# xwhan/ProQA

Hardware: AMD Instinct MI355X
Metric: queries/sec top-80 MIPS over 18M x 128 index (higher is better)
Workload: dtype int8 nomination + f16 re-scoring; 1 GPU; top-80 MIPS, 2032 q x 18000000 x 128 fp16 rows in HBM (BASELINE configs[2]; x1 row shards: co...; rows=18000000, queries=2032, topk=80, parallelism=corpus-row-shard x1, exchange=none, rounds=4, fallback_rounds=0, leap_rank=33, world_size=1

## Files before the change

### proqa_amd/csrc/mips_index.cpp

```cpp
#include <algorithm>
#include <cmath>
#include <cstdio>
#include <cstdlib>
#include <cstring>
#include <condition_variable>
#include <mutex>
#include <new>
#include <thread>
#include <vector>

#include <fcntl.h>
#include <unistd.h>
#include <cerrno>

#include "common.h"
#include "mips_kernels.h"

namespace proqa {

struct Slab {
  long long r0, r1;
};

}
// ... 1291 lines not shown
      log_line("index %p: a leaping round found fewer than k rows above its threshold or overflowed (%d overflow-safe rounds, overflow "
               "bits %u): ordinary rounds for the next %d searches", (void*)idx, idx->stats.fallback_rounds, idx->overflow_bits,
               idx->leap_skip);
    } else {
      log_line("index %p: a leaping round found fewer than k rows above its threshold for %zu quer%s: leaps go on (%d strikes of 8)",
               (void*)idx, idx->rescue.ids.size(), idx->rescue.ids.size() == 1 ? "y" : "ies", idx->leap_strikes);
    }
  } else {
    if (idx->leap_strikes > 0) --idx->leap_strikes;
    if (idx->leap_pause) {
      log_line("index %p: leaping rounds resumed", (void*)idx);
      idx->leap_pause = 0;
    }
  }
  idx->stats.leap_state = leap_state_of(idx);
}

int finish_pending(proqa_index* idx, int* rewritten);
int search_device_impl(proqa_index* idx, const void* xq_dev, int64_t nq, int dtype, int k, int64_t idx_offset, float* D_dev,
                       int64_t* I_dev, hipStream_t st, bool defer, uint32_t* status_dev);

int rescue_short_queries(proqa_index* idx) {
  proqa_index::Rescue rq;
  std::swap(rq, idx->rescue);
  const int s = (int)rq.ids.size(), k = rq.k;
  if (s == 0) return PROQA_OK;
  const size_t off_xq = round_up<size_t>((size_t)s * sizeof(int), 256), off_d = off_xq + (size_t)s * kDim * 2,
               off_i = round_up<size_t>(off_d + (size_t)s * k * sizeof(float), 256), bytes = off_i + (size_t)s * k * sizeof(long long);
  if (bytes > idx->rescue_bytes) {
    if (idx->rescue_buf) (void)hipFree(idx->rescue_buf);
  if (idx->emit_log) (void)hipFree(idx->emit_log);
  if (idx->emit_cnt) (void)hipFree(idx->emit_cnt);
    idx->rescue_buf = nullptr;
    idx->rescue_bytes = 0;
    PROQA_HIP(hipMalloc(&idx->rescue_buf, bytes));
    idx->rescue_bytes = bytes;
  }
  char* base = (char*)idx->rescue_buf;
  int* ids_dev = (int*)base;
  float* D_tmp = (float*)(base + off_d);
  long long* I_tmp = (long long*)(base + off_i);
  PROQA_HIP(hipMemcpyAsync(ids_dev, rq.ids.data(), (size_t)s * sizeof(int), hipMemcpyHostToDevice, rq.st));
  PROQA_HIP(launch_gather_query_rows(idx->xq_pad, ids_dev, s, base + off_xq, rq.st));
  const proqa_search_stats outer = idx->stats;
  const int mode = idx->leap_mode;
  idx->leap_mode = 0;
  const bool unprofitable = idx->q8_unprofitable, small_ok = idx->small_merge_ok;
  const int suspended = idx->q8_suspended_searches, probe_after = idx->q8_probe_after, on_copy = idx->q8_searches_on_copy;
  const int rc = search_device_impl(idx, base + off_xq, s, PROQA_F16, k, rq.idx_offset, D_tmp, (int64_t*)I_tmp, rq.st, false, nullptr);
  idx->leap_mode = mode;
  idx->q8_unprofitable = unprofitable;
  idx->small_merge_ok = small_ok;
  idx->q8_suspended_searches = suspended;
  idx->q8_probe_after = probe_after;
  idx->q8_searches_on_copy = on_copy;
  if (rc) return rc;
  PROQA_HIP(launch_scatter_result_rows(D_tmp, I_tmp, ids_dev, s, k, rq.D, rq.I, rq.out_stride, rq.st));
  PROQA_HIP(hipStreamSynchronize(rq.st));
  const proqa_search_stats inner = idx->stats;
  idx->stats = outer;
  idx->stats.fallback_rounds += inner.rounds + inner.fallback_rounds;
  idx->stats.candidates += inner.candidates;
  idx->stats.nominated += inner.nominated;
  idx->stats.total_ms += inner.total_ms;
  idx->stats.nomination_state = nomination_state_of(idx);
  idx->stats.leap_state = leap_state_of(idx);
  log_line("index %p: %d quer%s a leaping round left short searched again on ordinary rounds (%d rounds, %.3f ms)", (void*)idx, s,
           s == 1 ? "y" : "ies", inner.rounds, inner.total_ms);
  return PROQA_OK;
}

int search_device_impl_body(proqa_index* idx, const void* xq_dev, int64_t nq, int dtype, int k, int64_t idx_offset, float* D_dev,
                            int64_t* I_dev, hipStream_t st, bool defer, uint32_t* status_dev);

int search_device(proqa_index* idx, const void* xq_dev, int64_t nq, int dtype, int k, int64_t idx_offset,
                  float* D_dev, int64_t* I_dev, hipStream_t st, bool defer = false, uint32_t* status_dev = nullptr) {
  const int rc = search_device_impl(idx, xq_dev, nq, dtype, k, idx_offset, D_dev, I_dev, st, defer, status_dev);
#ifdef PROQA_FILTER_STAMPS
  {
    unsigned long long h[8];
    read_filter_stamps(h);
    if (h[4])
      fprintf(stderr, "filter stamps (one wave per workgroup, %llu workgroups over all launches of the search): per unit MFMA section %.1f "
              "ticks, test section %.1f ticks; units per wave %.0f, wave lifetime per unit %.1f ticks; int8 scan: barrier + DMA issue %.1f "
              "ticks per unit, %.3f excursions per unit of %.1f ticks each\n", h[4], (double)h[0] / h[2],
              (double)h[1] / h[2], (double)h[2] / h[4], (double)h[3] / h[2], (double)h[5] / h[2], (double)h[7] / h[2],
              h[7] ? (double)h[6] / h[7] : 0.0);
  }
#endif
  if (rc == PROQA_OK && status_dev && !idx->pending.active) PROQA_HIP(hipMemsetAsync(status_dev, 0, sizeof(uint32_t), st));
  return rc;
}

int search_device_impl(proqa_index* idx, const void* xq_dev, int64_t nq, int dtype, int k, int64_t idx_offset,
                       float* D_dev, int64_t* I_dev, hipStream_t st, bool defer, uint32_t* status_dev) {
  idx->rescue.ids.clear();
  if (int rc = search_device_impl_body(idx, xq_dev, nq, dtype, k, idx_offset, D_dev, I_dev, st, defer, status_dev)) return rc;
  return idx->rescue.ids.empty() ? PROQA_OK : rescue_short_queries(idx);
}

int search_device_impl_body(proqa_index* idx, const void* xq_dev, int64_t nq, int dtype, int k, int64_t idx_offset,
                            float* D_dev, int64_t* I_dev, hipStream_t st, bool defer, uint32_t* status_dev) {
  if (idx->pending.active)
    if (int rc = finish_pending(idx, nullptr)) return rc;
  if (nq < 0 || k <= 0) return fail(PROQA_EINVAL, "search: nq=%lld k=%d", (long long)nq, k);
  if (dtype != PROQA_F16 && dtype != PROQA_F32) return fail(PROQA_EINVAL, "search: bad dtype %d", dtype);
  if (idx->n >= (1ll << 32)) return fail(PROQA_EINVAL, "search: shard has >= 2^32 rows");
  idx->stats = {};
  idx->stats.nomination_state = nomination_state_of(idx);
  idx->stats.leap_state = leap_state_of(idx);
  idx->q8_active = false;
  idx->pending_nq = nq;
  idx->used_small_merge = false;
  idx->overflow_bits = 0;
  idx->leap_active = false;
  if (nq == 0) return PROQA_OK;
  PROQA_ON_DEVICE(idx->device);

  const int qw = nq > 256 ? 2 : 1;
  const unsigned tile_q = filter_tile_queries(qw);
  const unsigned n_qtiles = (unsigned)ceil_div<int64_t>(nq, tile_q);
  const int64_t nq_pad = (int64_t)n_qtiles * tile_q;
  const int page_size = k <= kPageK ? kPageK : kBigPageK;
  OnePassPlan one_pass = plan_one_pass(idx, nq_pad, k, qw == 1);
  if (one_pass.use && nq_pad > one_pass.max_queries) {
    const size_t esize = dtype == PROQA_F16 ? 2 : 4;
    proqa_search_stats sum = {};
    const int64_t n_groups = ceil_div<int64_t>(nq, one_pass.max_queries);
    const int64_t per_group = round_up<int64_t>(ceil_div<int64_t>(nq, n_groups), 512);
    for (int64_t q0 = 0; q0 < nq; q0 += per_group) {
      const int64_t m = std::min<int64_t>(per_group, nq - q0);
      if (int rc = search_device(idx, (const char*)xq_dev + (size_t)q0 * kDim * esize, m, dtype, k, idx_offset,
                                 D_dev + (size_t)q0 * k, I_dev + (size_t)q0 * k, st))
        return rc;
      sum.rounds += idx->stats.rounds;
      sum.fallback_rounds += idx->stats.fallback_rounds;
      sum.candidates += idx->stats.candidates;
      sum.filter_ms += idx->stats.filter_ms;
      sum.total_ms += idx->stats.total_ms;
    }
    idx->stats = sum;
    return PROQA_OK;
  }
  if (int rc = ensure_workspace(idx, nq_pad, one_pass.use ? k : std::min(k, page_size))) return rc;

  PROQA_HIP(hipEventRecord(idx->ev[0], st));
  int fallback = 0;
  auto prep_first = [&]() -> int {
    const bool check_q = dtype == PROQA_F32;
    if (check_q) PROQA_HIP(hipMemsetAsync(idx->inexact, 0, 2 * sizeof(unsigned), st));
    PROQA_HIP(launch_prep_queries(xq_dev, dtype, nq, idx->ws_nq_pad, idx->xq_pad, idx->tau, idx->run_n, idx->stat_dev,
                                  nullptr, true, check_q ? idx->inexact : nullptr, idx->overflow, st, idx->short_rounds));
    if (check_q) {
      unsigned bad = 0;
      if (int rc = read_inexact(idx, "index_search (queries)", st, &bad)) return rc;
      if (bad && !idx->allow_rounding)
        if (int rc = enable_exact(idx, st)) return rc;
    }
    return PROQA_OK;
  };
  auto setup_nominate = [&]() -> int {
    if (!nomination_eligible(idx, k)) return PROQA_OK;
    if (idx->q8_epoch != idx->rows_epoch) {
      if (idx->q8_searches_on_copy > 1) idx->q8_short_lived_builds = 0;
      if (idx->nominate_mode == 1 && idx->q8_short_lived_builds >= 2 && idx->q8_seen_epoch != idx->rows_epoch) {
        idx->q8_seen_epoch = idx->rows_epoch;
        log_line("index %p: rows changed again after an int8 copy that served %d search(es): this search scans the fp16 rows, the "
                 "copy is rebuilt when the rows stay", (void*)idx, idx->q8_searches_on_copy);
        return PROQA_OK;
      }
// ... 579 lines not shown
```

### proqa_amd/csrc/mips_kernels.h

```cpp
#pragma once
#include <hip/hip_runtime.h>
#include <stdint.h>

#include "../../include/proqa_hip.h"

namespace proqa {

constexpr int kDim = PROQA_EMBED_DIM;
constexpr int kFilterWaves = 8;
constexpr int kFilterThreads = kFilterWaves * 64;
__host__ __device__ constexpr unsigned filter_tile_queries(int qw) { return (unsigned)kFilterWaves * (unsigned)qw * 32u; }
constexpr int kStageRows = 128;
constexpr int kMergeThreads = 256;
constexpr int kMaxMergeListKeys = 16384;
constexpr int kMaxSortKeys = 2048;
constexpr int kPageK = kMaxSortKeys / 2;
constexpr int kBigSortKeys = 8192;
constexpr int kMidSortKeys = 4096;
constexpr int kBigPageK = kBigSortKeys / 2;
constexpr int kOnePassSortKeys = 16384;
constexpr int kOnePassMergeThreads = 1024;
constexpr int kOnePassLaneCap = 24;
constexpr int kLaneCap = 8;
constexpr int kBigLaneCap = 32;
// ... 30 lines not shown
constexpr unsigned kCompactKeys = 64;
static_assert(kCompactKeys <= kCompactLaneCap * kKeysPerRecord, "compact list size");

struct FilterArgs {
  const void* xq;
  const char* xb;
  long long slab_row0;
  long long slab_row1;
  int rows_per_chunk;
  const float* tau;
  const float* ub;
  CandidateStore store;
  unsigned* overflow;
  int compact;
};

struct MergeArgs {
  CandidateStore store;
  unsigned n_chunks;
  unsigned qw;
  unsigned long long* run_keys;
  unsigned* run_n;
  float* tau;
  int k;
  int sort_cap;
  int inclusive;
  const unsigned long long* bound_keys;
  unsigned long long* stat_candidates;
  unsigned* overflow;
  const float* xq32;
  const float* xb32;
  const float* margin;
  float* tau_filter;
  unsigned long long* dbg;
  int compact;
  int nom_keys;
  const void* xq16;
  const char* xb16;
  unsigned long long* stat_nominated;
  int next_rank;
  int leap_check;
  unsigned* short_rounds;
  int round_bit;
};

constexpr int kStageBytesI8 = kStageRows * kDim;
struct NominateParams {
  float off;
  float inv_unit;
  float margin_r;
  float err_norm;
};
static_assert(sizeof(NominateParams) == 16, "one 16-byte load per lane");
struct QuantStats {
  unsigned max_resid;
  unsigned max_inorm;
  unsigned max_xnorm;
  unsigned nonfinite;
};
struct FilterArgsI8 {
  const signed char* xq8;
  const signed char* xb8;
  long long slab_row0;
  long long slab_row1;
  int rows_per_chunk;
  const float* tau;
  const NominateParams* qp;
  const float2* blk;
  CandidateStore store;
  unsigned* overflow;
  unsigned q_blocks;
};
hipError_t launch_filter_i8(const FilterArgsI8& a, int qw, unsigned grid, hipStream_t st);
constexpr int kColStatGroups = 1024;
hipError_t launch_column_stats(const void* xb16, long long n, float* partial, float* col, QuantStats* stats, hipStream_t st);
hipError_t launch_quantise_rows_i8(const void* xb16, long long n, const float* col, signed char* xb8, float2* blk, QuantStats* stats,
                                   hipStream_t st);
hipError_t launch_prep_queries_i8(const void* xq_pad16, long long nq_pad, const float* col, const QuantStats* stats,
                                  signed char* xq8, NominateParams* qp, unsigned long long* stat_nom, hipStream_t st);

hipError_t launch_filter(const FilterArgs& a, int qw, bool inclusive, unsigned grid, hipStream_t st);
#ifdef PROQA_FILTER_STAMPS
void read_filter_stamps(unsigned long long* out5);
#endif
hipError_t launch_advance_page(const unsigned long long* run_keys, const unsigned* run_n, long long nq, int page_k,
                               unsigned long long* bound_keys, float* ub, unsigned char* done, const float* margin,
                               float* ub_filter, hipStream_t st);
hipError_t launch_merge(const MergeArgs& a, unsigned nq_pad, hipStream_t st);
hipError_t launch_gather_index_rows(const void* xb16, const float* xb32, long long n_index, const long long* ids, long long n,
                                    long long idx_offset, void* out, bool out_f32, hipStream_t st);
hipError_t launch_flag_short_lists(const unsigned* run_n, long long nq, unsigned want, unsigned* flag, hipStream_t st);
hipError_t launch_bootstrap(const char* xb, const void* xq_pad, int n_rows, unsigned nq_pad, int k, float* scores,
                            unsigned long long* run_keys, unsigned* run_n, float* tau, unsigned long long* stat,
                            unsigned* overflow, hipStream_t st, int run_stride = 0, int tau_rank = 0);
hipError_t launch_prep_queries(const void* xq, int dtype, long long nq, long long nq_pad, void* xq_pad,
                               float* tau, unsigned* run_n, unsigned long long* stat, const unsigned char* done,
                               bool reset_stat, unsigned* inexact, unsigned* overflow, hipStream_t st,
                               unsigned* short_rounds = nullptr);
struct RescoreArgs {
  CandidateStore in;
  unsigned in_lists;
  unsigned lists_per_group;
  CandidateStore out;
  const void* xq16;
  const char* xb16;
  const float* tau;
  unsigned* overflow;
  unsigned long long* stat_nominated;
};
hipError_t launch_rescore_nominated_lists(const RescoreArgs& a, unsigned groups, unsigned nq, hipStream_t st);
hipError_t launch_gather_query_rows(const void* xq_pad, const int* ids, int n, void* out, hipStream_t st);
hipError_t launch_scatter_result_rows(const float* D_src, const long long* I_src, const int* ids, int n, int k, float* D, long long* I,
                                      int out_stride, hipStream_t st);
constexpr int kOverflowWords = 96;
struct SearchMirror {
  unsigned overflow[kOverflowWords];
  unsigned long long candidates;
  unsigned long long nominated;
};
hipError_t launch_finalize(const unsigned long long* run_keys, const unsigned* run_n, long long nq, int page_k,
                           long long idx_offset, float* D, long long* I, int out_stride, int out_offset,
                           const unsigned* overflow, unsigned* status, SearchMirror* mirror, const unsigned long long* stat,
                           hipStream_t st, const unsigned long long* stat_nominated = nullptr);
hipError_t launch_merge_lists(const float* D_parts, const long long* I_parts, int n_parts, long long nq,
                              int k, long long stride_d, long long stride_i, float* D, long long* I, hipStream_t st,
                              const unsigned* status_src = nullptr, long long status_stride = 0, unsigned* status_host = nullptr,
                              bool parts_sorted = true);
hipError_t launch_convert_f32_to_f16(const float* src, void* dst, long long n, unsigned* inexact, hipStream_t st);
hipError_t launch_upconvert_f16_to_f32(const void* src, float* dst, long long n, hipStream_t st);
hipError_t launch_row_norm_stats(const float* xb32, const void* xb16, long long n_rows, unsigned* norm_stats,
                                 hipStream_t st);
hipError_t launch_query_margins(const void* xq, int dtype, long long nq, long long nq_pad, const unsigned* norm_stats,
                                float* xq32, float* margin, const float* tau, float* tau_filter, hipStream_t st);

}
```

### proqa_amd/csrc/mips_kernels.hip

```cpp
#include <hip/hip_runtime.h>
#include <algorithm>
#include <hipcub/hipcub.hpp>
#include <stdint.h>
#include <stdlib.h>

#include <type_traits>

#include "common.h"
#include "mips_kernels.h"

namespace proqa {
namespace {

typedef _Float16 f16x8 __attribute__((ext_vector_type(8)));
typedef float f32x16 __attribute__((ext_vector_type(16)));
typedef float f32x4 __attribute__((ext_vector_type(4)));

constexpr int kRowBytes = kDim * 2;
constexpr int kStageBytes = kStageRows * kRowBytes;
constexpr int kSubRows = 32;
#ifndef PROQA_DMA_AUX
#define PROQA_DMA_AUX 2
#endif
constexpr int kDmaAux = PROQA_DMA_AUX;
constexpr int kSubBytes = kSubRows * kRowBytes;

__device__ __forceinline__ unsigned ord_from_float(float f) {
  unsigned u = __float_as_uint(f);
  if (u == 0x80000000u) u = 0u;
  return (u & 0x80000000u) ? ~u : (u | 0x80000000u);
}
__device__ __forceinline__ float float_from_ord(unsigned o) {
  unsigned u = (o & 0x80000000u) ? (o & 0x7fffffffu) : ~o;
  return __uint_as_float(u);
}
__device__ __forceinline__ unsigned long long pack_key(float score, unsigned row) {
  return ((unsigned long long)ord_from_float(score) << 32) | (unsigned long long)(0xFFFFFFFFu - row);
}

__device__ __forceinline__ float max3_f32(float a, float b, float c) {
  float r;
  asm("v_max3_f32 %0, %1, %2, %3" : "=v"(r) : "v"(a), "v"(b), "v"(c));
  return r;
}

__device__ __forceinline__ float max4_f32(float a, float b, float c, float d) {
  float r;
  asm("v_max3_f32 %0, %1, %2, %3\n\tv_max_f32 %0, %0, %4" : "=&v"(r) : "v"(a), "v"(b), "v"(c), "v"(d));
  return r;
}
__device__ __forceinline__ float max16_f32(const float (&v)[16]) {
  float r;
  asm("v_max3_f32 %0, %1, %2, %3\n\t"
      "v_max3_f32 %0, %0, %4, %5\n\t"
      "v_max3_f32 %0, %0, %6, %7\n\t"
      "v_max3_f32 %0, %0, %8, %9\n\t"
      "v_max3_f32 %0, %0, %10, %11\n\t"
      "v_max3_f32 %0, %0, %12, %13\n\t"
      "v_max3_f32 %0, %0, %14, %15\n\t"
      "v_max_f32 %0, %0, %16"
      : "=&v"(r)
      : "v"(v[0]), "v"(v[1]), "v"(v[2]), "v"(v[3]), "v"(v[4]), "v"(v[5]), "v"(v[6]), "v"(v[7]), "v"(v[8]), "v"(v[9]), "v"(v[10]),
        "v"(v[11]), "v"(v[12]), "v"(v[13]), "v"(v[14]), "v"(v[15]));
  return r;
}

__device__ __forceinline__ unsigned gt_mask16_f32(const f32x16& v, float thr) {
  unsigned mask = 0u;
#define PROQA_BIT(n) "v_cmp_gt_f32 vcc, %" #n ", %17\n\tv_addc_co_u32 %0, vcc, %0, %0, vcc\n\t"
  asm volatile(PROQA_BIT(16) PROQA_BIT(15) PROQA_BIT(14) PROQA_BIT(13) PROQA_BIT(12) PROQA_BIT(11) PROQA_BIT(10) PROQA_BIT(9)
               PROQA_BIT(8) PROQA_BIT(7) PROQA_BIT(6) PROQA_BIT(5) PROQA_BIT(4) PROQA_BIT(3) PROQA_BIT(2) PROQA_BIT(1)
               : "+v"(mask)
               : "v"(v[0]), "v"(v[1]), "v"(v[2]), "v"(v[3]), "v"(v[4]), "v"(v[5]), "v"(v[6]), "v"(v[7]), "v"(v[8]), "v"(v[9]),
                 "v"(v[10]), "v"(v[11]), "v"(v[12]), "v"(v[13]), "v"(v[14]), "v"(v[15]), "v"(thr)
               : "vcc");
#undef PROQA_BIT
  return mask;
}

__device__ __forceinline__ float max2_f32(float a, float b) {
  float r;
  asm("v_max_f32 %0, %1, %2" : "=v"(r) : "v"(a), "v"(b));
  return r;
}

__device__ __forceinline__ size_t lane_list_index(const CandidateStore& st, unsigned chunk, unsigned q, int half) {
  return ((size_t)chunk * st.nq_pad + q) * 2 + half;
}
__device__ __forceinline__ size_t lane_cnt_index(const CandidateStore& st, unsigned chunk, unsigned q, int half) {
  return ((size_t)q * st.n_chunks + chunk) * 2 + half;
}
__device__ __forceinline__ size_t spill_cnt_index(const CandidateStore& st, unsigned chunk, unsigned qt, unsigned wave) {
  return ((size_t)qt * kFilterWaves + wave) * st.n_chunks + chunk;
}

#ifdef PROQA_FILTER_STAMPS
__device__ unsigned long long g_filter_stamps[8];
#endif
__device__ __forceinline__ void write_record(WaveRecord* dst, const f32x16& acc, unsigned q, unsigned row0,
                                             int rows_left, float tau) {
  uint4* d = (uint4*)dst;
  d[0] = make_uint4(q, row0, (unsigned)rows_left, __float_as_uint(tau));
#pragma unroll
  for (int g = 0; g < 4; ++g)
    d[1 + g] = make_uint4(__float_as_uint(acc[4 * g]), __float_as_uint(acc[4 * g + 1]),
                          __float_as_uint(acc[4 * g + 2]), __float_as_uint(acc[4 * g + 3]));
}

template <int QW, bool INCLUSIVE, bool BOUNDED, bool COMPACT = false>
__global__ __launch_bounds__(kFilterThreads) void mips_filter_f16(FilterArgs a) {
  static_assert(QW == 1 || QW == 2, "8 waves x 32 or 64 queries");
  static_assert(!COMPACT || (!INCLUSIVE && !BOUNDED), "compact lists: first page, strict threshold only");
  __shared__ __attribute__((aligned(16))) char lds[4 * kStageBytes];

  const int tid = threadIdx.x;
  const int lane = tid & 63;
  const int wave = __builtin_amdgcn_readfirstlane(tid >> 6);
  const int li = lane & 31;
  const int half = lane >> 5;

  const unsigned b = blockIdx.x;
  const unsigned xcd = b & 7u;
  const unsigned rest = b >> 3;
  const unsigned qt = rest % a.store.n_qtiles;
  const unsigned grp = rest / a.store.n_qtiles;
  const unsigned chunk = grp * 8 + xcd;
  const long long row_begin = a.slab_row0 + (long long)chunk * a.rows_per_chunk;
  if (row_begin >= a.slab_row1) return;
  long long row_end = row_begin + a.rows_per_chunk;
  if (row_end > a.slab_row1) row_end = a.slab_row1;
  const int n_rows = (int)(row_end - row_begin);
  const int nstages = (n_rows + kStageRows - 1) / kStageRows;
  const unsigned row_begin32 = (unsigned)row_begin;
  const char* chunk_base = a.xb + row_begin * kRowBytes;

  const unsigned q0 = qt * (kFilterWaves * QW * 32) + wave * (QW * 32);
  f16x8 qf[QW][8];
  float tau[QW];
  float ub[QW];
  WaveRecord* lane_list[QW];
  unsigned lane_n[QW];
#pragma unroll
  for (int blk = 0; blk < QW; ++blk) {
    const unsigned q = q0 + blk * 32 + li;
    const char* qrow = (const char*)a.xq + (size_t)q * kRowBytes;
#pragma unroll
    for (int j = 0; j < 8; ++j) qf[blk][j] = *(const f16x8*)(qrow + (2 * j + half) * 16);
    tau[blk] = a.tau[q];
    ub[blk] = BOUNDED ? a.ub[q] : 0.f;
    lane_n[blk] = 0u;
    lane_list[blk] = a.store.lane_log + lane_list_index(a.store, chunk, q, half) * a.store.lane_cap;
  }
  const unsigned wave_slot = (chunk * a.store.n_qtiles + qt) * kFilterWaves + wave;
  WaveRecord* spill_log = a.store.spill_log + (size_t)wave_slot * kSpillCap;
  int spill_n = 0;

  unsigned rd_off[8];
#pragma unroll
  for (int j = 0; j < 8; ++j) rd_off[j] = li * kRowBytes + (((2 * j + half) ^ (li & 15)) << 4);

  constexpr int kDmaPerWave = 32 / kFilterWaves;
  const int dma_row = lane >> 4;
  const int dma_slot = lane & 15;
  int dma_rel[kDmaPerWave];
  int dma_piece_off[kDmaPerWave];
#pragma unroll
  for (int e = 0; e < kDmaPerWave; ++e) {
    dma_rel[e] = (wave * kDmaPerWave + e) * 4 + dma_row;
    dma_piece_off[e] = (dma_slot ^ (dma_rel[e] & 15)) * 16;
  }
  auto issue_stage = [&](int s, int buf_off) {
#pragma unroll
    for (int e = 0; e < kDmaPerWave; ++e) {
      int rel = s * kStageRows + dma_rel[e];
      rel = rel < n_rows ? rel : n_rows - 1;
      const char* src = chunk_base + (long long)rel * kRowBytes + dma_piece_off[e];
      __builtin_amdgcn_global_load_lds((const __attribute__((address_space(1))) void*)src,
                                       (__attribute__((address_space(3))) void*)(lds + buf_off + (wave * kDmaPerWave + e) * 1024),
                                       16, 0, QW == 1 ? kDmaAux : 0);
    }
// ... 283 lines not shown
  const int ti = thr < -2147483000.f ? (int)0x80000000 : (int)__builtin_floorf(thr);
  unsigned mask = 0u;
#define PROQA_BIT(n) "v_cmp_gt_i32 vcc, %" #n ", %17\n\tv_addc_co_u32 %0, vcc, %0, %0, vcc\n\t"
  asm volatile(PROQA_BIT(16) PROQA_BIT(15) PROQA_BIT(14) PROQA_BIT(13) PROQA_BIT(12) PROQA_BIT(11) PROQA_BIT(10) PROQA_BIT(9)
               PROQA_BIT(8) PROQA_BIT(7) PROQA_BIT(6) PROQA_BIT(5) PROQA_BIT(4) PROQA_BIT(3) PROQA_BIT(2) PROQA_BIT(1)
               : "+v"(mask)
               : "v"(acc[0]), "v"(acc[1]), "v"(acc[2]), "v"(acc[3]), "v"(acc[4]), "v"(acc[5]), "v"(acc[6]), "v"(acc[7]), "v"(acc[8]),
                 "v"(acc[9]), "v"(acc[10]), "v"(acc[11]), "v"(acc[12]), "v"(acc[13]), "v"(acc[14]), "v"(acc[15]), "v"(ti)
               : "vcc");
#undef PROQA_BIT
  return mask;
}
__device__ __forceinline__ unsigned column_rows_mask(int rows_left) {
  unsigned valid = 0u;
#pragma unroll
  for (int g = 0; g < 4; ++g) {
    const int c = rows_left - 8 * g;
    valid |= (c >= 4 ? 0xFu : (c > 0 ? (1u << c) - 1u : 0u)) << (4 * g);
  }
  return valid;
}

template <int QW, bool SPLIT = false>
__global__ __launch_bounds__(kFilterThreads, 2) void mips_filter_i8(FilterArgsI8 a) {
  static_assert(QW == 1 || QW == 2, "8 waves x 32 / 64 queries");
  static_assert(!SPLIT || QW == 1, "row-split launches keep one query block per wave");
  __shared__ __attribute__((aligned(16))) char lds[4 * kStageBytesI8];
  constexpr int NW = kFilterWaves;
  const int tid = threadIdx.x;
  const int lane = tid & 63;
  const int wave = __builtin_amdgcn_readfirstlane(tid >> 6);
  const int li = lane & 31;
  const int half = lane >> 5;

  const unsigned b = blockIdx.x;
  const unsigned xcd = b & 7u;
  const unsigned rest = b >> 3;
  const unsigned qt = rest % a.store.n_qtiles;
  const unsigned grp = rest / a.store.n_qtiles;
  const unsigned chunk = grp * 8 + xcd;
  const long long row_begin = a.slab_row0 + (long long)chunk * a.rows_per_chunk;
  if (row_begin >= a.slab_row1) return;
  long long row_end = row_begin + a.rows_per_chunk;
  if (row_end > a.slab_row1) row_end = a.slab_row1;
  const int n_rows = (int)(row_end - row_begin);
  const int nstages = (n_rows + kStageRows - 1) / kStageRows;
  const int npairs = (nstages + 1) / 2;
  const unsigned row_begin32 = (unsigned)row_begin;
  const signed char* chunk_base = a.xb8 + row_begin * kRowBytesI8;

  const unsigned n_qblk = SPLIT ? a.q_blocks : (unsigned)NW;
  const unsigned n_slices = (unsigned)NW / n_qblk;
  const unsigned qwave = SPLIT ? (unsigned)wave % n_qblk : (unsigned)wave;
  const unsigned slice = SPLIT ? (unsigned)wave / n_qblk : 0u;
  __shared__ unsigned s_list_n[SPLIT ? 4 * 64 : 1];
  if constexpr (SPLIT) {
    if (tid < 4 * 64) s_list_n[tid] = 0u;
  }
  const unsigned q0 = SPLIT ? qwave * 32u : qt * (NW * QW * 32) + wave * (QW * 32);
  i32x4 qf[QW][4];
  LaneThreshold thr[QW];
  uint2* lane_list[QW];
  unsigned lane_n[QW];
  bool wave_live = false;
#pragma unroll
  for (int blk = 0; blk < QW; ++blk) {
    const unsigned q = q0 + blk * 32 + li;
    const signed char* qrow = a.xq8 + (size_t)q * kRowBytesI8;
#pragma unroll
    for (int j = 0; j < 4; ++j) qf[blk][j] = *(const i32x4*)(qrow + (2 * j + half) * 16);
    thr[blk] = lane_threshold(a.tau[q], a.qp[q]);
    wave_live = wave_live || thr[blk].A != __builtin_inff();
    lane_n[blk] = 0u;
    lane_list[blk] = (uint2*)a.store.lane_log + lane_list_index(a.store, chunk, q, half) * a.store.lane_cap;
  }
  wave_live = __any(wave_live);
  const unsigned lane_cap = a.store.lane_cap;

  unsigned rd_off[4];
#pragma unroll
  for (int j = 0; j < 4; ++j) rd_off[j] = li * kRowBytesI8 + (((2 * j + half) ^ ((li >> 1) & 7)) << 4);

  constexpr int kDmaPerWave = (kStageBytesI8 / 1024) / NW;
  int dma_rel[kDmaPerWave];
  int dma_piece_off[kDmaPerWave];
#pragma unroll
  for (int e = 0; e < kDmaPerWave; ++e) {
    dma_rel[e] = (wave * kDmaPerWave + e) * 8 + (lane >> 3);
    dma_piece_off[e] = ((lane & 7) ^ ((dma_rel[e] >> 1) & 7)) * 16;
  }
  auto issue_pair = [&](int p) {
#pragma unroll
    for (int h = 0; h < 2; ++h) {
      const int s = 2 * p + h;
      if (s < nstages) {
#pragma unroll
        for (int e = 0; e < kDmaPerWave; ++e) {
          int rel = s * kStageRows + dma_rel[e];
          rel = rel < n_rows ? rel : n_rows - 1;
          const signed char* src = chunk_base + (long long)rel * kRowBytesI8 + dma_piece_off[e];
          __builtin_amdgcn_global_load_lds((const __attribute__((address_space(1))) void*)src,
                                           (__attribute__((address_space(3))) void*)(lds + ((p & 1) * 2 + h) * kStageBytesI8 +
                                                                                     (wave * kDmaPerWave + e) * 1024),
                                           16, 0, QW == 1 ? kDmaAux : 0);
        }
      }
    }
  };
  int st_cur = 0;
  auto publish = [&]() {
    const int allowed = __builtin_amdgcn_readfirstlane(st_cur);
    if (allowed >= 8) {
      asm volatile("s_waitcnt vmcnt(8)" ::: "memory");
    } else if (allowed >= 6) {
      asm volatile("s_waitcnt vmcnt(6)" ::: "memory");
    } else if (allowed >= 4) {
      asm volatile("s_waitcnt vmcnt(4)" ::: "memory");
    } else if (allowed >= 3) {
      asm volatile("s_waitcnt vmcnt(3)" ::: "memory");
    } else if (allowed >= 2) {
      asm volatile("s_waitcnt vmcnt(2)" ::: "memory");
    } else if (allowed >= 1) {
      asm volatile("s_waitcnt vmcnt(1)" ::: "memory");
    } else {
      asm volatile("s_waitcnt vmcnt(0)" ::: "memory");
    }
    asm volatile("s_waitcnt lgkmcnt(0)" ::: "memory");
    __builtin_amdgcn_s_barrier();
    asm volatile("" ::: "memory");
    st_cur = 0;
  };
  if (npairs > 0) issue_pair(0);
  if (!wave_live) {
    for (int p = 0; p < npairs; ++p) {
      publish();
      if (p + 1 < npairs) issue_pair(p + 1);
    }
  }
  auto load_blocks = [&](int p) {
    const unsigned long long addr = (unsigned long long)(a.blk + (row_begin >> 5) + 8ll * p);
    const unsigned lo = (unsigned)__builtin_amdgcn_readfirstlane((int)(unsigned)addr);
    const unsigned hi = (unsigned)__builtin_amdgcn_readfirstlane((int)(unsigned)(addr >> 32));
    const unsigned long long uaddr = ((unsigned long long)hi << 32) | lo;
    return *(const __attribute__((address_space(4))) f32x16*)uaddr;
  };
  for (int p = 0; wave_live && p < npairs; ++p) {
    const f32x16 bc = load_blocks(p);
    publish();
    if (p + 1 < npairs) issue_pair(p + 1);
    const char* base = lds + (p & 1) * 2 * kStageBytesI8;
    const int nunits = (nstages - 2 * p >= 2 ? 2 : 1) * (kStageRows / kSubRows);
    i32x4 af[4];
    if constexpr (!SPLIT) {
#pragma unroll
      for (int j = 0; j < 4; ++j) af[j] = *(const i32x4*)(base + rd_off[j]);
    }
#pragma unroll
    for (int u = 0; u < 8; ++u) {
      if (u == 4 && nunits <= 4) break;
      if constexpr (SPLIT) {
        if (((unsigned)u & (n_slices - 1u)) != slice) continue;
#pragma unroll
        for (int j = 0; j < 4; ++j) af[j] = *(const i32x4*)(base + u * kSubBytesI8 + rd_off[j]);
      }
      const char* nxt = base + (u + 1 < nunits ? u + 1 : u) * kSubBytesI8;
      i32x16 acc[QW];
#pragma unroll
      for (int blk = 0; blk < QW; ++blk) acc[blk] = i32x16{0};
#pragma unroll
      for (int j = 0; j < 4; ++j) {
#pragma unroll
        for (int blk = 0; blk < QW; ++blk)
          acc[blk] = __builtin_amdgcn_mfma_i32_32x32x32_i8(af[j], qf[blk][j], acc[blk], 0, 0, 0);
      }
      if constexpr (!SPLIT) {
#pragma unroll
        for (int j = 0; j < 4; ++j) af[j] = *(const i32x4*)(nxt + rd_off[j]);
      }
      bool hit[QW];
      float tb[QW];
      bool any_hit = false;
#pragma unroll
      for (int blk = 0; blk < QW; ++blk) {
        tb[blk] = block_threshold(thr[blk], bc[2 * u], bc[2 * u + 1]);
        hit[blk] = (float)max16_i32(acc[blk]) > tb[blk];
        any_hit = any_hit || hit[blk];
      }
      if (__builtin_expect(__any(any_hit), 0)) {
        int rel0 = (2 * p * 4 + u) * kSubRows;
        asm volatile("" : "+v"(rel0));
        const int rel = rel0 + 4 * half;
#pragma unroll
        for (int blk = 0; blk < QW; ++blk) {
          if (__any(hit[blk])) {
            st_cur += 1;
            if (hit[blk]) {
              unsigned pos = lane_n[blk];
              if constexpr (SPLIT) {
                const unsigned addr = (unsigned)(size_t)(__attribute__((address_space(3))) unsigned*)&s_list_n[qwave * 64u + (unsigned)lane];
                asm volatile("ds_add_rtn_u32 %0, %1, %2\n\ts_waitcnt lgkmcnt(0)" : "=&v"(pos) : "v"(addr), "v"(1u) : "memory");
              }
              const unsigned slot = pos < lane_cap ? pos : lane_cap - 1u;
              unsigned mask = nominee_mask(acc[blk], tb[blk]);
#ifdef PROQA_TAILMASK_HOISTED
              if ((2 * p * 4 + u + 1) * kSubRows > n_rows) mask &= column_rows_mask(n_rows - rel);
#else
              if ((2 * p * 4 + u + 1) * kSubRows > n_rows) {
                int rows_left = n_rows - rel;
                asm volatile("" : "+v"(rows_left));
                mask &= column_rows_mask(rows_left);
              }
#endif
              lane_list[blk][slot] = make_uint2(row_begin32 + (unsigned)rel, mask);
              ++lane_n[blk];
            }
          }
        }
      }
    }
  }
  if constexpr (SPLIT) {
    asm volatile("s_waitcnt lgkmcnt(0)" ::: "memory");
    __builtin_amdgcn_s_barrier();
    asm volatile("" ::: "memory");
    if (slice == 0) {
      lane_n[0] = s_list_n[qwave * 64u + (unsigned)lane];
    } else {
      a.store.lane_cnt[lane_cnt_index(a.store, chunk, (unsigned)wave * 32u + li, half)] = 0u;
      return;
    }
  }
#pragma unroll
  for (int blk = 0; blk < QW; ++blk) {
    if (lane_n[blk] > lane_cap) {
      *a.overflow = 1u;
      lane_n[blk] = lane_cap;
    }
    a.store.lane_cnt[lane_cnt_index(a.store, chunk, q0 + blk * 32 + li, half)] = lane_n[blk];
  }
}

__device__ __forceinline__ float wave_sum_f(float v) {
#pragma unroll
  for (int off = 32; off > 0; off >>= 1) v += __shfl_xor(v, off, 64);
  return v;
}
__device__ __forceinline__ float wave_max_f(float v) {
#pragma unroll
  for (int off = 32; off > 0; off >>= 1) v = __builtin_fmaxf(v, __shfl_xor(v, off, 64));
  return v;
}

__global__ __launch_bounds__(256) void column_stats_partial(const _Float16* __restrict__ xb, long long n, float* __restrict__ partial,
                                                            QuantStats* __restrict__ stats) {
  __shared__ float red[3][16][kDim];
  const int lane = threadIdx.x & 63, w = threadIdx.x >> 6;
  const int sub = lane & 15, slot = w * 4 + (lane >> 4);
  float sum[8], lo[8], hi[8];
#pragma unroll
  for (int e = 0; e < 8; ++e) {
    sum[e] = 0.f;
    lo[e] = __builtin_inff();
    hi[e] = -__builtin_inff();
  }
  bool bad = false;
  for (long long r = (long long)blockIdx.x * 16 + slot; r < n; r += (long long)gridDim.x * 16) {
    const f16x8 v = *(const f16x8*)(xb + r * kDim + sub * 8);
#pragma unroll
    for (int e = 0; e < 8; ++e) {
      const float x = (float)v[e];
      bad = bad || !(__builtin_fabsf(x) < __builtin_inff());
      sum[e] += x;
      lo[e] = __builtin_fminf(lo[e], x);
      hi[e] = __builtin_fmaxf(hi[e], x);
    }
  }
  if (bad) atomicOr(&stats->nonfinite, 1u);
#pragma unroll
  for (int e = 0; e < 8; ++e) {
    red[0][slot][sub * 8 + e] = sum[e];
    red[1][slot][sub * 8 + e] = lo[e];
    red[2][slot][sub * 8 + e] = hi[e];
  }
  __syncthreads();
  if (threadIdx.x < kDim) {
    const int d = threadIdx.x;
    float s_ = 0.f, l_ = __builtin_inff(), h_ = -__builtin_inff();
#pragma unroll
    for (int t = 0; t < 16; ++t) {
      s_ += red[0][t][d];
      l_ = __builtin_fminf(l_, red[1][t][d]);
      h_ = __builtin_fmaxf(h_, red[2][t][d]);
    }
    float* out = partial + (size_t)blockIdx.x * 3 * kDim;
    out[d] = s_;
    out[kDim + d] = l_;
    out[2 * kDim + d] = h_;
  }
}

__global__ __launch_bounds__(kDim) void column_stats_finish(const float* __restrict__ partial, int groups, long long n, float* __restrict__ col,
                                                            QuantStats* __restrict__ stats) {
  const int d = threadIdx.x;
// ... 1431 lines not shown
    const unsigned p = pos / k, jj = pos - p * k;
    D[q * k + j] = float_from_ord((unsigned)(key >> 32));
    I[q * k + j] = I_parts[(size_t)p * stride_i + (size_t)q * k + jj];
  } else {
    D[q * k + j] = -3.4028234663852886e38f;
    I[q * k + j] = -1;
  }
}

}

template <int QW, bool INCLUSIVE>
static void launch_filter_bounded(const FilterArgs& a, dim3 g, hipStream_t st) {
  if (a.ub)
    hipLaunchKernelGGL((mips_filter_f16<QW, INCLUSIVE, true>), g, dim3(kFilterThreads), 0, st, a);
  else
    hipLaunchKernelGGL((mips_filter_f16<QW, INCLUSIVE, false>), g, dim3(kFilterThreads), 0, st, a);
}

hipError_t launch_filter(const FilterArgs& a, int qw, bool inclusive, unsigned grid, hipStream_t st) {
  dim3 g(grid);
  if (a.compact) {
    if (qw != 2 || inclusive || a.ub) return hipErrorInvalidValue;
    hipLaunchKernelGGL((mips_filter_f16<2, false, false, true>), g, dim3(kFilterThreads), 0, st, a);
    return hipGetLastError();
  }
  if (qw == 2) {
    if (inclusive)
      launch_filter_bounded<2, true>(a, g, st);
    else
      launch_filter_bounded<2, false>(a, g, st);
  } else {
    if (inclusive)
      launch_filter_bounded<1, true>(a, g, st);
    else
      launch_filter_bounded<1, false>(a, g, st);
  }
  return hipGetLastError();
}

hipError_t launch_filter_i8(const FilterArgsI8& a, int qw, unsigned grid, hipStream_t st) {
  if (qw == 2)
    hipLaunchKernelGGL((mips_filter_i8<2>), dim3(grid), dim3(kFilterThreads), 0, st, a);
  else if (qw == 1 && a.q_blocks) {
    if (a.q_blocks != 1 && a.q_blocks != 2 && a.q_blocks != 4) return hipErrorInvalidValue;
    hipLaunchKernelGGL((mips_filter_i8<1, true>), dim3(grid), dim3(kFilterThreads), 0, st, a);
  } else if (qw == 1)
    hipLaunchKernelGGL((mips_filter_i8<1>), dim3(grid), dim3(kFilterThreads), 0, st, a);
  else
    return hipErrorInvalidValue;
  return hipGetLastError();
}

hipError_t launch_column_stats(const void* xb16, long long n, float* partial, float* col, QuantStats* stats, hipStream_t st) {
  hipLaunchKernelGGL(column_stats_partial, dim3(kColStatGroups), dim3(256), 0, st, (const _Float16*)xb16, n, partial, stats);
  hipLaunchKernelGGL(column_stats_finish, dim3(1), dim3(kDim), 0, st, partial, kColStatGroups, n, col, stats);
  return hipGetLastError();
}

hipError_t launch_quantise_rows_i8(const void* xb16, long long n, const float* col, signed char* xb8, float2* blk, QuantStats* stats,
                                   hipStream_t st) {
  if (n == 0) return hipSuccess;
  const long long want = ((n + 31) / 32 + 3) / 4;
  const unsigned grid = (unsigned)std::min<long long>(want, 8ll * 1024);
  hipLaunchKernelGGL(quantise_rows_i8, dim3(grid), dim3(256), 0, st, (const _Float16*)xb16, n, col, xb8, blk, stats);
  return hipGetLastError();
}

hipError_t launch_prep_queries_i8(const void* xq_pad16, long long nq_pad, const float* col, const QuantStats* stats,
                                  signed char* xq8, NominateParams* qp, unsigned long long* stat_nom, hipStream_t st) {
  if (nq_pad == 0) return hipSuccess;
  hipLaunchKernelGGL(prep_queries_i8, dim3((unsigned)((nq_pad + 3) / 4)), dim3(256), 0, st, (const _Float16*)xq_pad16, nq_pad, col,
                     stats, xq8, qp, stat_nom);
  return hipGetLastError();
}

#ifdef PROQA_FILTER_STAMPS
void read_filter_stamps(unsigned long long* out5) {
  (void)hipDeviceSynchronize();
  (void)hipMemcpyFromSymbol(out5, HIP_SYMBOL(g_filter_stamps), 8 * sizeof(unsigned long long));
  unsigned long long z[8] = {};
  (void)hipMemcpyToSymbol(HIP_SYMBOL(g_filter_stamps), z, sizeof z);
}
#endif

hipError_t launch_advance_page(const unsigned long long* run_keys, const unsigned* run_n, long long nq, int page_k,
                               unsigned long long* bound_keys, float* ub, unsigned char* done, const float* margin,
                               float* ub_filter, hipStream_t st) {
  hipLaunchKernelGGL(advance_page, dim3((unsigned)((nq + 255) / 256)), dim3(256), 0, st, run_keys, run_n, nq, page_k,
                     bound_keys, ub, done, margin, ub_filter);
  return hipGetLastError();
}

hipError_t launch_upconvert_f16_to_f32(const void* src, float* dst, long long n, hipStream_t st) {
  if (n == 0) return hipSuccess;
  const long long nthreads = (n + 7) / 8;
  hipLaunchKernelGGL(upconvert_rows_f16_to_f32, dim3((unsigned)((nthreads + 255) / 256)), dim3(256), 0, st,
                     (const _Float16*)src, dst, n);
  return hipGetLastError();
}

hipError_t launch_row_norm_stats(const float* xb32, const void* xb16, long long n_rows, unsigned* norm_stats,
                                 hipStream_t st) {
  if (n_rows == 0) return hipSuccess;
  hipLaunchKernelGGL(row_norm_stats, dim3((unsigned)((n_rows + 3) / 4)), dim3(256), 0, st, xb32,
                     (const _Float16*)xb16, n_rows, norm_stats);
  return hipGetLastError();
}

hipError_t launch_query_margins(const void* xq, int dtype, long long nq, long long nq_pad, const unsigned* norm_stats,
                                float* xq32, float* margin, const float* tau, float* tau_filter, hipStream_t st) {
  if (nq_pad == 0) return hipSuccess;
  hipLaunchKernelGGL(query_margins, dim3((unsigned)((nq_pad + 3) / 4)), dim3(256), 0, st, xq, dtype, nq, nq_pad,
                     norm_stats, xq32, margin, tau, tau_filter);
  return hipGetLastError();
}

hipError_t launch_bootstrap(const char* xb, const void* xq_pad, int n_rows, unsigned nq_pad, int k, float* scores,
                            unsigned long long* run_keys, unsigned* run_n, float* tau, unsigned long long* stat,
                            unsigned* overflow, hipStream_t st, int run_stride, int tau_rank) {
  if (run_stride <= 0) run_stride = k;
  if (tau_rank <= 0 || tau_rank > k) tau_rank = k;
  const int s_stride = (n_rows + 31) / 32 * 32;
  const unsigned row_tiles = (unsigned)(s_stride / 32);
  const unsigned per_wg = kBootWaves * kBootTilesPerWave;
  hipLaunchKernelGGL(bootstrap_scores, dim3((row_tiles + per_wg - 1) / per_wg, nq_pad / 32), dim3(kBootWaves * 64), 0, st,
                     xb, xq_pad, n_rows, s_stride, scores);
#define PROQA_SELECT_CASE(E)                                                                                            \
  hipLaunchKernelGGL(bootstrap_select<E>, dim3(nq_pad), dim3(kMergeThreads), 0, st, scores, n_rows, s_stride, k, run_stride, \
                     run_keys, run_n, tau, stat, overflow, tau_rank)
  if (n_rows <= 4 * kMergeThreads)
    PROQA_SELECT_CASE(4);
  else if (n_rows <= 8 * kMergeThreads)
    PROQA_SELECT_CASE(8);
  else if (n_rows <= 16 * kMergeThreads)
    PROQA_SELECT_CASE(16);
  else
    PROQA_SELECT_CASE(32);
#undef PROQA_SELECT_CASE
  static_assert(kBootstrapMaxRows == 32 * kMergeThreads, "largest select");
  return hipGetLastError();
}

hipError_t launch_gather_index_rows(const void* xb16, const float* xb32, long long n_index, const long long* ids, long long n,
                                    long long idx_offset, void* out, bool out_f32, hipStream_t st) {
  if (n == 0) return hipSuccess;
  const long long pieces = n * (out_f32 ? kDim / 4 : kDim / 8);
  hipLaunchKernelGGL(gather_index_rows, dim3((unsigned)((pieces + 255) / 256)), dim3(256), 0, st, (const _Float16*)xb16, xb32,
                     n_index, ids, n, idx_offset, out, out_f32 ? 1 : 0);
  return hipGetLastError();
}

hipError_t launch_rescore_nominated_lists(const RescoreArgs& a, unsigned groups, unsigned nq, hipStream_t st) {
  if (groups == 0 || nq == 0) return hipSuccess;
  if (a.lists_per_group == 0 || a.lists_per_group > 64) return hipErrorInvalidValue;
  hipLaunchKernelGGL(rescore_nominated_lists, dim3(groups, nq), dim3(256), 0, st, a);
  return hipGetLastError();
}

hipError_t launch_gather_query_rows(const void* xq_pad, const int* ids, int n, void* out, hipStream_t st) {
  if (n == 0) return hipSuccess;
  hipLaunchKernelGGL(gather_query_rows, dim3((unsigned)((n * (kRowBytes / 16) + 255) / 256)), dim3(256), 0, st, (const uint4*)xq_pad, ids, n,
                     (uint4*)out);
  return hipGetLastError();
}
hipError_t launch_scatter_result_rows(const float* D_src, const long long* I_src, const int* ids, int n, int k, float* D, long long* I,
// ... 155 lines not shown
```

Before: 493,900 queries/s.

## Interleave next-pair DMA issue with MFMA units and raise priority on hit path

After: 496,300 queries/s (median of 6 runs). No clear change (+0.5%).

```diff
diff --git a/proqa_amd/csrc/mips_index.cpp b/proqa_amd/csrc/mips_index.cpp
--- a/proqa_amd/csrc/mips_index.cpp
+++ b/proqa_amd/csrc/mips_index.cpp
@@ -1397,10 +1397,34 @@
     read_filter_stamps(h);
     if (h[4])
       fprintf(stderr, "filter stamps (one wave per workgroup, %llu workgroups over all launches of the search): per unit MFMA section %.1f "
-              "ticks, test section %.1f ticks; units per wave %.0f, wave lifetime per unit %.1f ticks; int8 scan: barrier + DMA issue %.1f "
-              "ticks per unit, %.3f excursions per unit of %.1f ticks each\n", h[4], (double)h[0] / h[2],
-              (double)h[1] / h[2], (double)h[2] / h[4], (double)h[3] / h[2], (double)h[5] / h[2], (double)h[7] / h[2],
-              h[7] ? (double)h[6] / h[7] : 0.0);
+              "ticks, test section %.1f ticks; units per wave %.0f, wave lifetime per unit %.1f ticks\n", h[4], (double)h[0] / h[2],
+              (double)h[1] / h[2], (double)h[2] / h[4], (double)h[3] / h[2]);
+    std::vector<unsigned long long> w((size_t)kFilterI8StampSlots * 8);
+    read_filter_i8_stamps(w.data());
+    std::vector<double> seg[6];
+    for (unsigned s = 0; s < kFilterI8StampSlots; ++s) {
+      const unsigned long long* v = &w[(size_t)s * 8];
+      if (!v[5]) continue;
+      const double pairs = (double)v[5];
+      seg[0].push_back(v[0] / pairs);
+      seg[1].push_back(v[1] / pairs);
+      seg[2].push_back(((double)v[4] - v[0] - v[1] - v[2]) / pairs);
+      seg[3].push_back(v[2] / pairs);
+      seg[4].push_back(v[3] / pairs);
+      if (v[3]) seg[5].push_back((double)v[2] / v[3]);
+    }
+    if (!seg[0].empty()) {
+      auto q = [](std::vector<double>& d, double f) {
+        if (d.empty()) return 0.0;
+        std::sort(d.begin(), d.end());
+        return d[(size_t)(f * (d.size() - 1))];
+      };
+      fprintf(stderr, "int8 filter stamps (%zu waves, s_memtime ticks per pair and wave, median [p10, p90]): publish wait %.0f [%.0f, %.0f], "
+              "DMA issue %.0f [%.0f, %.0f], units %.0f [%.0f, %.0f], hit path %.0f [%.0f, %.0f]; excursions per pair %.2f [%.2f, %.2f] of "
+              "%.0f [%.0f, %.0f] ticks each\n", seg[0].size(), q(seg[0], .5), q(seg[0], .1), q(seg[0], .9), q(seg[1], .5), q(seg[1], .1),
+              q(seg[1], .9), q(seg[2], .5), q(seg[2], .1), q(seg[2], .9), q(seg[3], .5), q(seg[3], .1), q(seg[3], .9), q(seg[4], .5),
+              q(seg[4], .1), q(seg[4], .9), q(seg[5], .5), q(seg[5], .1), q(seg[5], .9));
+    }
   }
 #endif
   if (rc == PROQA_OK && status_dev && !idx->pending.active) PROQA_HIP(hipMemsetAsync(status_dev, 0, sizeof(uint32_t), st));
diff --git a/proqa_amd/csrc/mips_kernels.h b/proqa_amd/csrc/mips_kernels.h
--- a/proqa_amd/csrc/mips_kernels.h
+++ b/proqa_amd/csrc/mips_kernels.h
@@ -136,6 +136,8 @@
 hipError_t launch_filter(const FilterArgs& a, int qw, bool inclusive, unsigned grid, hipStream_t st);
 #ifdef PROQA_FILTER_STAMPS
 void read_filter_stamps(unsigned long long* out5);
+constexpr unsigned kFilterI8StampSlots = 16384;
+void read_filter_i8_stamps(unsigned long long* out);
 #endif
 hipError_t launch_advance_page(const unsigned long long* run_keys, const unsigned* run_n, long long nq, int page_k,
                                unsigned long long* bound_keys, float* ub, unsigned char* done, const float* margin,
diff --git a/proqa_amd/csrc/mips_kernels.hip b/proqa_amd/csrc/mips_kernels.hip
--- a/proqa_amd/csrc/mips_kernels.hip
+++ b/proqa_amd/csrc/mips_kernels.hip
@@ -96,6 +96,42 @@
 
 #ifdef PROQA_FILTER_STAMPS
 __device__ unsigned long long g_filter_stamps[8];
+__device__ unsigned long long g_filter_i8_stamps[kFilterI8StampSlots * 8];
+struct I8Stamps {
+  unsigned long long t = 0, t0 = 0, wait = 0, dma = 0, exc = 0, n_exc = 0;
+  __device__ __forceinline__ static unsigned long long now() {
+    __builtin_amdgcn_sched_barrier(0);
+    const unsigned long long v = __builtin_amdgcn_s_memtime();
+    __builtin_amdgcn_sched_barrier(0);
+    return v;
+  }
+  __device__ __forceinline__ void start() { t0 = now(); }
+  __device__ __forceinline__ void begin() { t = now(); }
+  __device__ __forceinline__ void end(unsigned long long& segment) { segment += now() - t; }
+  __device__ __forceinline__ void end_excursion() {
+    end(exc);
+    ++n_exc;
+  }
+  __device__ __forceinline__ void report(bool reporter, int npairs, int wave) {
+    if (!reporter) return;
+    unsigned long long* slot = g_filter_i8_stamps + ((blockIdx.x * 8u + (unsigned)wave) % kFilterI8StampSlots) * 8;
+    atomicAdd(slot + 0, wait);
+    atomicAdd(slot + 1, dma);
+    atomicAdd(slot + 2, exc);
+    atomicAdd(slot + 3, n_exc);
+    atomicAdd(slot + 4, now() - t0);
+    atomicAdd(slot + 5, (unsigned long long)npairs);
+  }
+};
+#else
+struct I8Stamps {
+  int wait = 0, dma = 0;
+  __device__ __forceinline__ void start() {}
+  __device__ __forceinline__ void begin() {}
+  __device__ __forceinline__ void end(int&) {}
+  __device__ __forceinline__ void end_excursion() {}
+  __device__ __forceinline__ void report(bool, int, int) {}
+};
 #endif
 __device__ __forceinline__ void write_record(WaveRecord* dst, const f32x16& acc, unsigned q, unsigned row0,
                                              int rows_left, float tau) {
@@ -545,31 +581,39 @@
   for (int j = 0; j < 4; ++j) rd_off[j] = li * kRowBytesI8 + (((2 * j + half) ^ ((li >> 1) & 7)) << 4);
 
   constexpr int kDmaPerWave = (kStageBytesI8 / 1024) / NW;
-  int dma_rel[kDmaPerWave];
-  int dma_piece_off[kDmaPerWave];
+  unsigned dma_off[kDmaPerWave];
 #pragma unroll
   for (int e = 0; e < kDmaPerWave; ++e) {
-    dma_rel[e] = (wave * kDmaPerWave + e) * 8 + (lane >> 3);
-    dma_piece_off[e] = ((lane & 7) ^ ((dma_rel[e] >> 1) & 7)) * 16;
-  }
+    const int r = (wave * kDmaPerWave + e) * 8 + (lane >> 3);
+    dma_off[e] = (unsigned)(r * kRowBytesI8 + (((lane & 7) ^ ((r >> 1) & 7)) * 16));
+  }
+  const bool ragged = (n_rows & (kStageRows - 1)) != 0;
+  auto issue_piece = [&](int p, int i, const signed char* pair_src) {
+    const int h = i >> 1, e = i & 1;
+    const int s = 2 * p + h;
+    if (s >= nstages) return;
+    auto* dst = (__attribute__((address_space(3))) void*)(lds + ((p & 1) * 2 + h) * kStageBytesI8 + (wave * kDmaPerWave + e) * 1024);
+    if (ragged && s == nstages - 1) {
+      int rel = s * kStageRows + (int)(dma_off[e] >> 7);
+      asm volatile("" : "+v"(rel));
+      rel = rel < n_rows ? rel : n_rows - 1;
+      const signed char* src = chunk_base + (long long)rel * kRowBytesI8 + (dma_off[e] & (unsigned)(kRowBytesI8 - 1));
+      __builtin_amdgcn_global_load_lds((const __attribute__((address_space(1))) void*)src, dst, 16, 0, QW == 1 ? kDmaAux : 0);
+      asm volatile("");
+    } else {
+      const unsigned long long sa = (unsigned long long)(pair_src + h * kStageBytesI8);
+      const unsigned lo = (unsigned)__builtin_amdgcn_readfirstlane((int)(unsigned)sa);
+      const unsigned hi = (unsigned)__builtin_amdgcn_readfirstlane((int)(unsigned)(sa >> 32));
+      const signed char* src = (const signed char*)(((unsigned long long)hi << 32) | lo) + dma_off[e];
+      __builtin_amdgcn_global_load_lds((const __attribute__((address_space(1))) void*)src, dst, 16, 0, QW == 1 ? kDmaAux : 0);
+    }
+  };
   auto issue_pair = [&](int p) {
-#pragma unroll
-    for (int h = 0; h < 2; ++h) {
-      const int s = 2 * p + h;
-      if (s < nstages) {
-#pragma unroll
-        for (int e = 0; e < kDmaPerWave; ++e) {
-          int rel = s * kStageRows + dma_rel[e];
-          rel = rel < n_rows ? rel : n_rows - 1;
-          const signed char* src = chunk_base + (long long)rel * kRowBytesI8 + dma_piece_off[e];
-          __builtin_amdgcn_global_load_lds((const __attribute__((address_space(1))) void*)src,
-                                           (__attribute__((address_space(3))) void*)(lds + ((p & 1) * 2 + h) * kStageBytesI8 +
-                                                                                     (wave * kDmaPerWave + e) * 1024),
-                                           16, 0, QW == 1 ? kDmaAux : 0);
-        }
-      }
-    }
+    const signed char* pair_src = chunk_base + (long long)p * (2 * kStageBytesI8);
+#pragma unroll
+    for (int i = 0; i < 2 * kDmaPerWave; ++i) issue_piece(p, i, pair_src);
   };
+  I8Stamps stamps;
   int st_cur = 0;
   auto publish = [&]() {
     const int allowed = __builtin_amdgcn_readfirstlane(st_cur);
@@ -591,7 +635,6 @@
     asm volatile("s_waitcnt lgkmcnt(0)" ::: "memory");
     __builtin_amdgcn_s_barrier();
     asm volatile("" ::: "memory");
-    st_cur = 0;
   };
   if (npairs > 0) issue_pair(0);
   if (!wave_live) {
@@ -607,10 +650,13 @@
     const unsigned long long uaddr = ((unsigned long long)hi << 32) | lo;
     return *(const __attribute__((address_space(4))) f32x16*)uaddr;
   };
-  for (int p = 0; wave_live && p < npairs; ++p) {
+  const signed char* next_src = chunk_base + 2 * kStageBytesI8;
+  stamps.start();
+  for (int p = 0; wave_live && p < npairs; ++p, next_src += 2 * kStageBytesI8) {
     const f32x16 bc = load_blocks(p);
+    stamps.begin();
     publish();
-    if (p + 1 < npairs) issue_pair(p + 1);
+    stamps.end(stamps.wait);
     const char* base = lds + (p & 1) * 2 * kStageBytesI8;
     const int nunits = (nstages - 2 * p >= 2 ? 2 : 1) * (kStageRows / kSubRows);
     i32x4 af[4];
@@ -621,7 +667,14 @@
 #pragma unroll
     for (int u = 0; u < 8; ++u) {
       if (u == 4 && nunits <= 4) break;
+      auto next_piece = [&]() {
+        stamps.begin();
+        issue_piece(p + 1, u, next_src);
+        if (u == 3) st_cur = 0;
+        stamps.end(stamps.dma);
+      };
       if constexpr (SPLIT) {
+        if (u < 4) next_piece();
         if (((unsigned)u & (n_slices - 1u)) != slice) continue;
 #pragma unroll
         for (int j = 0; j < 4; ++j) af[j] = *(const i32x4*)(base + u * kSubBytesI8 + rd_off[j]);
@@ -650,6 +703,8 @@
         any_hit = any_hit || hit[blk];
       }
       if (__builtin_expect(__any(any_hit), 0)) {
+        __builtin_amdgcn_s_setprio(3);
+        stamps.begin();
         int rel0 = (2 * p * 4 + u) * kSubRows;
         asm volatile("" : "+v"(rel0));
         const int rel = rel0 + 4 * half;
@@ -679,9 +734,15 @@
             }
           }
         }
-      }
-    }
-  }
+        stamps.end_excursion();
+        __builtin_amdgcn_s_setprio(0);
+      }
+      if constexpr (!SPLIT) {
+        if (u < 4) next_piece();
+      }
+    }
+  }
+  stamps.report(wave_live && lane == 0, npairs, wave);
   if constexpr (SPLIT) {
     asm volatile("s_waitcnt lgkmcnt(0)" ::: "memory");
     __builtin_amdgcn_s_barrier();
@@ -2279,6 +2340,13 @@
   unsigned long long z[8] = {};
   (void)hipMemcpyToSymbol(HIP_SYMBOL(g_filter_stamps), z, sizeof z);
 }
+void read_filter_i8_stamps(unsigned long long* out) {
+  (void)hipDeviceSynchronize();
+  (void)hipMemcpyFromSymbol(out, HIP_SYMBOL(g_filter_i8_stamps), sizeof(unsigned long long) * kFilterI8StampSlots * 8);
+  void* dev = nullptr;
+  (void)hipGetSymbolAddress(&dev, HIP_SYMBOL(g_filter_i8_stamps));
+  (void)hipMemset(dev, 0, sizeof(unsigned long long) * kFilterI8StampSlots * 8);
+}
 #endif
 
 hipError_t launch_advance_page(const unsigned long long* run_keys, const unsigned* run_n, long long nq, int page_k,
```
